# zjkang/Relation-DETR

Measured on AMD Instinct MI355X. Metric: images/sec @ 800×1333, 300 queries, R50 4-level; achieved HBM GB/s, higher is better.
Workload: dtype bf16; 1 GPU; relation_detr_resnet50_800_1333 transformer stack from feature pyramids: 6 encoder layers (MSDA self-attn, S=22323, 4 levels) + two-stage top-k + 6 decoder layers (relation-biased self-attn + MSDA cross-attn + box refinement) + top-300 detections; backbone/neck excluded; batch_per_gpu=4, global_batch=4, queries=900, levels=4, launch=hipGraph replay, streams=2, gemm_tuning=False, parallelism=image-parallel x1

## Files before the change

### relation_detr_amd/csrc/linear.hip

```cpp
#include <cstdlib>

#include "common.h"

namespace rdetr {

typedef __bf16 ln_bf16x8 __attribute__((ext_vector_type(8)));

constexpr int kLinK = 256;
constexpr int kLinThreads = 512;
constexpr int kLinRows = 32;

template <int NT, bool RELU>
__global__ __launch_bounds__(kLinThreads) void linear_k256_kernel(const uint16_t *__restrict__ x, long long ldx,
                                                                  const uint16_t *__restrict__ w, const uint16_t *__restrict__ bias,
                                                                  long long M, int N, uint16_t *__restrict__ out, long long ldo, int dbg,
                                                                  const unsigned char *__restrict__ row_mask, int hm_S)
{
    extern __shared__ __attribute__((aligned(16))) unsigned char lin_lds[];
    u32x4 *wl = reinterpret_cast<u32x4 *>(lin_lds);
    float *bl = reinterpret_cast<float *>(lin_lds + NT * 8 * 64 * 16);
    const int tid = threadIdx.x, lane = tid & 63, wave = tid >> 6;
    const int col = lane & 15, g = lane >> 4;
    const int n0 = blockIdx.y * (NT * 16);

    {
        constexpr int kPer = NT * 16 * 32 / kLinThreads;
        u32x4 piece[kPer];
#pragma unroll
        for (int i = 0; i < kPer; ++i) {
            const int idx = i * kLinThreads + tid, c = idx >> 5, p = idx & 31;
            piece[i] = n0 + c < N ? *reinterpret_cast<const u32x4 *>(w + (size_t)(n0 + c) * kLinK + 8 * p) : u32x4{0u, 0u, 0u, 0u};
        }
#pragma unroll
        for (int i = 0; i < kPer; ++i) {
            const int idx = i * kLinThreads + tid, c = idx >> 5, p = idx & 31;
            const int t = 2 * (c >> 5) + ((c >> 2) & 1), m = 4 * ((c >> 3) & 3) + (c & 3);
            wl[(t * 8 + (p >> 2)) * 64 + 16 * (p & 3) + m] = piece[i];
        }
    }
    for (int i = tid; i < NT * 16; i += kLinThreads) bl[i] = (bias && n0 + i < N) ? bf16_bits_to_f32(bias[n0 + i]) : 0.f;
    __syncthreads();

    const long long nsteps = (M + kLinRows - 1) / kLinRows;
    constexpr int kWaves = kLinThreads / 64;
    const long long stride = (long long)gridDim.x * kWaves;
    long long step = (long long)blockIdx.x * kWaves + wave;

    u32x4 xc[2][8], xn[2][8];
    auto load_rows = [&](long long st, u32x4 (&dst)[2][8]) {
#pragma unroll
        for (int cb = 0; cb < 2; ++cb) {
            const long long row = st * kLinRows + cb * 16 + col;
            const uint16_t *p = x + row * ldx + 8 * g;
#pragma unroll
            for (int s = 0; s < 8; ++s)
                dst[cb][s] = (st < nsteps && row < M) ? *reinterpret_cast<const u32x4 *>(p + 32 * s) : u32x4{0u, 0u, 0u, 0u};
        }
    };
    load_rows(step, xc);
    for (; step < nsteps; step += stride) {
        load_rows(step + stride, xn);
        const long long row_a = step * kLinRows + col, row_b = row_a + 16;
        uint16_t *oa = out + row_a * ldo + n0 + 8 * g, *ob = out + row_b * ldo + n0 + 8 * g;
        bool zero_a = false, zero_b = false;
        if (hm_S) {
            const unsigned ia = (unsigned)row_a / (unsigned)hm_S, ib = (unsigned)row_b / (unsigned)hm_S;
            oa = out + ((long long)ia * 8 * hm_S + (row_a - (long long)ia * hm_S)) * 32 + 8 * g;
            ob = out + ((long long)ib * 8 * hm_S + (row_b - (long long)ib * hm_S)) * 32 + 8 * g;
            if (row_mask) {
                zero_a = row_a < M && row_mask[row_a] != 0;
                zero_b = row_b < M && row_mask[row_b] != 0;
            }
        }
#pragma unroll
        for (int u = 0; u < NT / 2; ++u) {
            f32x4 acc[2][2];
#pragma unroll
            for (int e = 0; e < 2; ++e) {
                const f32x4 b4 = *reinterpret_cast<const f32x4 *>(bl + 32 * u + 8 * g + 4 * e);
                acc[e][0] = b4;
                acc[e][1] = b4;
            }
            if (!(dbg & 2))
#pragma unroll
            for (int s = 0; s < 8; ++s) {
#pragma unroll
                for (int e = 0; e < 2; ++e) {
                    const ln_bf16x8 a = __builtin_bit_cast(ln_bf16x8, wl[((2 * u + e) * 8 + s) * 64 + lane]);
                    acc[e][0] = __builtin_amdgcn_mfma_f32_16x16x32_bf16(a, __builtin_bit_cast(ln_bf16x8, xc[0][s]), acc[e][0], 0, 0, 0);
                    acc[e][1] = __builtin_amdgcn_mfma_f32_16x16x32_bf16(a, __builtin_bit_cast(ln_bf16x8, xc[1][s]), acc[e][1], 0, 0, 0);
                }
            }
            if (n0 + 32 * u + 8 * g < N) {
#pragma unroll
                for (int cb = 0; cb < 2; ++cb) {
                    f32x4 lo = acc[0][cb], hi = acc[1][cb];
                    if (RELU) {
                        lo.x = fmaxf(lo.x, 0.f); lo.y = fmaxf(lo.y, 0.f); lo.z = fmaxf(lo.z, 0.f); lo.w = fmaxf(lo.w, 0.f);
                        hi.x = fmaxf(hi.x, 0.f); hi.y = fmaxf(hi.y, 0.f); hi.z = fmaxf(hi.z, 0.f); hi.w = fmaxf(hi.w, 0.f);
                    }
                    u32x4 pk;
                    pk.x = f32_to_bf16_bits(lo.x) | (f32_to_bf16_bits(lo.y) << 16);
                    pk.y = f32_to_bf16_bits(lo.z) | (f32_to_bf16_bits(lo.w) << 16);
                    pk.z = f32_to_bf16_bits(hi.x) | (f32_to_bf16_bits(hi.y) << 16);
                    pk.w = f32_to_bf16_bits(hi.z) | (f32_to_bf16_bits(hi.w) << 16);
                    if ((cb ? zero_b : zero_a)) pk = u32x4{0u, 0u, 0u, 0u};
                    const long long col_off = hm_S ? (long long)u * hm_S * 32 : 32 * u;
                    if ((cb ? row_b : row_a) < M && !((dbg & 1) && pk.x != 0x12345u)) *reinterpret_cast<u32x4 *>((cb ? ob : oa) + col_off) = pk;
                }
            }
            __builtin_amdgcn_sched_barrier(0);
        }
#pragma unroll
        for (int cb = 0; cb < 2; ++cb)
#pragma unroll
            for (int s = 0; s < 8; ++s) xc[cb][s] = xn[cb][s];
    }
}

template <int NT, bool RELU>
static int linear_launch(const uint16_t *x, long long ldx, const uint16_t *w, const uint16_t *bias, long long M, int N,
                         uint16_t *out, long long ldo, int chunks, hipStream_t st, const unsigned char *row_mask = nullptr, int hm_S = 0)
{
    auto kern = linear_k256_kernel<NT, RELU>;
    constexpr int lds = NT * 8 * 64 * 16 + NT * 16 * 4;
    static const hipError_t attr = hipFuncSetAttribute(reinterpret_cast<const void *>(kern),
                                                       hipFuncAttributeMaxDynamicSharedMemorySize, lds);
    if (attr != hipSuccess) return RDETR_ERR_LAUNCH;
    const long long steps = (M + kLinRows - 1) / kLinRows;
    long long gx = (steps + kLinThreads / 64 - 1) / (kLinThreads / 64);
    const long long cap = 256 / chunks > 0 ? 256 / chunks : 1;
    if (gx > cap) gx = cap;
    hipLaunchKernelGGL(kern, dim3((unsigned)gx, (unsigned)chunks), dim3(kLinThreads), (size_t)lds, st, x, ldx, w, bias, M, N, out,
                       ldo, 0, row_mask, hm_S);
    return launch_status();
}


constexpr int kLnlThreads = 512;
constexpr int kLnlWaves = kLnlThreads / 64;

__global__ __launch_bounds__(256) void linear_pack_kernel(const uint16_t *__restrict__ w, u32x4 *__restrict__ packed)
{
    const int idx = blockIdx.x * 256 + threadIdx.x;
    if (idx >= 16 * 8 * 64) return;
    const int t = idx >> 9, s = (idx >> 6) & 7, l = idx & 63, m = l & 15, kb = l >> 4;
    const int n = 32 * (t >> 1) + 8 * (m >> 2) + 4 * (t & 1) + (m & 3);
    packed[idx] = *reinterpret_cast<const u32x4 *>(w + (size_t)n * kLinK + 32 * s + 8 * kb);
}

__global__ __launch_bounds__(kLnlThreads) void linear_ln_k256_kernel(const uint16_t *__restrict__ x, long long ldx,
                                                                     const uint16_t *__restrict__ packed,
                                                                     const uint16_t *__restrict__ bias,
                                                                     const uint16_t *__restrict__ res, long long ldr,
                                                                     const uint16_t *__restrict__ gamma,
                                                                     const uint16_t *__restrict__ beta, float eps, long long M,
                                                                     uint16_t *__restrict__ out, long long ldo)
{
    extern __shared__ __attribute__((aligned(16))) unsigned char lin_lds[];
    const u32x4 *wl = reinterpret_cast<const u32x4 *>(lin_lds);
    float *bl = reinterpret_cast<float *>(lin_lds + 16 * 8 * 64 * 16);
    const int tid = threadIdx.x, lane = tid & 63, wave = __builtin_amdgcn_readfirstlane(tid >> 6);
    const int col = lane & 15, g = lane >> 4;
    {
        const unsigned lane_off = (unsigned)lane * 16u;
#pragma unroll 1
        for (int i = 0; i < 128 / kLnlWaves; ++i) {
            const int f = wave * (128 / kLnlWaves) + i;
            const unsigned m0v = (unsigned)f * 1024u;
            const unsigned char *src = reinterpret_cast<const unsigned char *>(packed) + f * 1024;
            asm volatile("s_mov_b32 m0, %0\n\ts_nop 0\n\tglobal_load_lds_dwordx4 %1, %2" : : "s"(m0v), "v"(lane_off), "s"(src) : "memory", "m0");
        }
    }
    if (tid < 256) {
        bl[tid] = bias ? bf16_bits_to_f32(bias[tid]) : 0.f;
        bl[256 + tid] = bf16_bits_to_f32(gamma[tid]);
        bl[512 + tid] = bf16_bits_to_f32(beta[tid]);
    }
    const long long nsteps = (M + kLinRows - 1) / kLinRows;
    long long step = (long long)blockIdx.x * kLnlWaves + wave;
    const long long stride = (long long)gridDim.x * kLnlWaves;
    asm volatile("s_waitcnt vmcnt(0)" ::: "memory");
    __syncthreads();
    for (; step < nsteps; step += stride) {
        const long long row_a = step * kLinRows + col, row_b = row_a + 16;
        u32x4 xc[2][8];
#pragma unroll
        for (int s = 0; s < 8; ++s) {
            xc[0][s] = row_a < M ? *reinterpret_cast<const u32x4 *>(x + row_a * ldx + 32 * s + 8 * g) : u32x4{0u, 0u, 0u, 0u};
            xc[1][s] = row_b < M ? *reinterpret_cast<const u32x4 *>(x + row_b * ldx + 32 * s + 8 * g) : u32x4{0u, 0u, 0u, 0u};
        }
        f32x4 acc[16][2];
        {
            auto frag = [&](int i) -> u32x4 { return wl[((i & 15) * 8 + (i >> 4)) * 64 + lane]; };
            const f32x4 zero4 = {0.f, 0.f, 0.f, 0.f};
            u32x4 ring[3];
            ring[0] = frag(0);
            ring[1] = frag(1);
#pragma unroll
            for (int i = 0; i < 128; ++i) {
                if (i + 2 < 128) ring[(i + 2) % 3] = frag(i + 2);
                __builtin_amdgcn_sched_barrier(0);
                const int s = i >> 4, t = i & 15;
                const ln_bf16x8 a = __builtin_bit_cast(ln_bf16x8, ring[i % 3]);
                acc[t][0] = __builtin_amdgcn_mfma_f32_16x16x32_bf16(a, __builtin_bit_cast(ln_bf16x8, xc[0][s]), s ? acc[t][0] : zero4, 0, 0, 0);
                acc[t][1] = __builtin_amdgcn_mfma_f32_16x16x32_bf16(a, __builtin_bit_cast(ln_bf16x8, xc[1][s]), s ? acc[t][1] : zero4, 0, 0, 0);
                __builtin_amdgcn_sched_barrier(0);
            }
        }
#pragma unroll
        for (int cb = 0; cb < 2; ++cb) {
            const long long row = cb ? row_b : row_a;
            const bool ok = row < M;
            float sum = 0.f;
#pragma unroll
            for (int u = 0; u < 8; ++u) {
                const u32x4 r = ok ? *reinterpret_cast<const u32x4 *>(res + row * ldr + 32 * u + 8 * g) : u32x4{0u, 0u, 0u, 0u};
                f32x4 &lo = acc[2 * u][cb], &hi = acc[2 * u + 1][cb];
                lo += *reinterpret_cast<const f32x4 *>(bl + 32 * u + 8 * g);
                hi += *reinterpret_cast<const f32x4 *>(bl + 32 * u + 8 * g + 4);
                const unsigned p0 = pack_bf16x2(lo.x, lo.y), p1 = pack_bf16x2(lo.z, lo.w), p2 = pack_bf16x2(hi.x, hi.y), p3 = pack_bf16x2(hi.z, hi.w);
                lo.x = __builtin_bit_cast(float, p0 << 16) + __builtin_bit_cast(float, r.x << 16);
                lo.y = __builtin_bit_cast(float, p0 & 0xffff0000u) + __builtin_bit_cast(float, r.x & 0xffff0000u);
                lo.z = __builtin_bit_cast(float, p1 << 16) + __builtin_bit_cast(float, r.y << 16);
                lo.w = __builtin_bit_cast(float, p1 & 0xffff0000u) + __builtin_bit_cast(float, r.y & 0xffff0000u);
                hi.x = __builtin_bit_cast(float, p2 << 16) + __builtin_bit_cast(float, r.z << 16);
                hi.y = __builtin_bit_cast(float, p2 & 0xffff0000u) + __builtin_bit_cast(float, r.z & 0xffff0000u);
                hi.z = __builtin_bit_cast(float, p3 << 16) + __builtin_bit_cast(float, r.w << 16);
                hi.w = __builtin_bit_cast(float, p3 & 0xffff0000u) + __builtin_bit_cast(float, r.w & 0xffff0000u);
                sum += ((lo.x + lo.y) + (lo.z + lo.w)) + ((hi.x + hi.y) + (hi.z + hi.w));
            }
            sum += __shfl_xor(sum, 16, 64);
            sum += __shfl_xor(sum, 32, 64);
            const float mean = sum * (1.0f / 256.0f);
            float sq = 0.f;
#pragma unroll
            for (int u = 0; u < 8; ++u) {
                f32x4 &lo = acc[2 * u][cb], &hi = acc[2 * u + 1][cb];
                lo.x -= mean; lo.y -= mean; lo.z -= mean; lo.w -= mean;
                hi.x -= mean; hi.y -= mean; hi.z -= mean; hi.w -= mean;
                sq += ((lo.x * lo.x + lo.y * lo.y) + (lo.z * lo.z + lo.w * lo.w)) + ((hi.x * hi.x + hi.y * hi.y) + (hi.z * hi.z + hi.w * hi.w));
            }
            sq += __shfl_xor(sq, 16, 64);
            sq += __shfl_xor(sq, 32, 64);
            const float rstd = 1.0f / sqrtf(sq * (1.0f / 256.0f) + eps);
#pragma unroll
            for (int u = 0; u < 8; ++u) {
                const f32x4 lo = acc[2 * u][cb], hi = acc[2 * u + 1][cb];
                const float *gp = bl + 256 + 32 * u + 8 * g, *bp = bl + 512 + 32 * u + 8 * g;
                const f32x4 g0 = *reinterpret_cast<const f32x4 *>(gp), g1 = *reinterpret_cast<const f32x4 *>(gp + 4);
                const f32x4 c0 = *reinterpret_cast<const f32x4 *>(bp), c1 = *reinterpret_cast<const f32x4 *>(bp + 4);
                u32x4 pk;
                pk.x = pack_bf16x2(lo.x * rstd * g0.x + c0.x, lo.y * rstd * g0.y + c0.y);
                pk.y = pack_bf16x2(lo.z * rstd * g0.z + c0.z, lo.w * rstd * g0.w + c0.w);
                pk.z = pack_bf16x2(hi.x * rstd * g1.x + c1.x, hi.y * rstd * g1.y + c1.y);
                pk.w = pack_bf16x2(hi.z * rstd * g1.z + c1.z, hi.w * rstd * g1.w + c1.w);
                if (ok) *reinterpret_cast<u32x4 *>(out + row * ldo + 32 * u + 8 * g) = pk;
            }
        }
    }
}

}

using namespace rdetr;

extern "C" int rdetr_linear_k256_bf16(const uint16_t *x, long long ldx, const uint16_t *w, const uint16_t *bias, long long M,
                                      int N, int relu, uint16_t *out, long long ldo, void *stream)
{
    if (M < 0 || N <= 0 || ldx < kLinK || ldo < N) return RDETR_ERR_INVALID_ARG;
    if ((N & 31) || (ldx & 7) || (ldo & 7)) return RDETR_ERR_UNSUPPORTED;
    if (M == 0) return RDETR_OK;
    if (!x || !w || !out) return RDETR_ERR_INVALID_ARG;
    if ((reinterpret_cast<uintptr_t>(x) | reinterpret_cast<uintptr_t>(w) | reinterpret_cast<uintptr_t>(out)) & 15) return RDETR_ERR_UNSUPPORTED;
    hipStream_t st = static_cast<hipStream_t>(stream);
    if (N % 256 == 0 || N < 192 || (N % 192 != 0)) {
        const int chunks = (N + 255) / 256;
        return relu ? linear_launch<16, true>(x, ldx, w, bias, M, N, out, ldo, chunks, st)
                    : linear_launch<16, false>(x, ldx, w, bias, M, N, out, ldo, chunks, st);
    }
    const int chunks = N / 192;
    return relu ? linear_launch<12, true>(x, ldx, w, bias, M, N, out, ldo, chunks, st)
                : linear_launch<12, false>(x, ldx, w, bias, M, N, out, ldo, chunks, st);
}

extern "C" int rdetr_linear_k256_hm_bf16(const uint16_t *x, long long ldx, const uint16_t *w, const uint16_t *bias,
                                         const uint8_t *row_mask, int B, int S, uint16_t *out_hm, void *stream)
{
    if (B < 0 || S < 0 || ldx < kLinK) return RDETR_ERR_INVALID_ARG;
    if (ldx & 7) return RDETR_ERR_UNSUPPORTED;
    if (B == 0 || S == 0) return RDETR_OK;
    if ((long long)B * S >= (1ll << 31)) return RDETR_ERR_UNSUPPORTED;
    if (!x || !w || !out_hm) return RDETR_ERR_INVALID_ARG;
    if ((reinterpret_cast<uintptr_t>(x) | reinterpret_cast<uintptr_t>(w) | reinterpret_cast<uintptr_t>(out_hm)) & 15) return RDETR_ERR_UNSUPPORTED;
    return linear_launch<16, false>(x, ldx, w, bias, (long long)B * S, 256, out_hm, 256, 1, static_cast<hipStream_t>(stream), row_mask, S);
}

extern "C" int rdetr_linear_pack_k256_bf16(const uint16_t *w, uint16_t *packed, void *stream)
{
    if (!w || !packed) return RDETR_ERR_INVALID_ARG;
    if ((reinterpret_cast<uintptr_t>(w) | reinterpret_cast<uintptr_t>(packed)) & 15) return RDETR_ERR_UNSUPPORTED;
    hipLaunchKernelGGL(linear_pack_kernel, dim3(32), dim3(256), 0, static_cast<hipStream_t>(stream), w, reinterpret_cast<u32x4 *>(packed));
    return launch_status();
}

extern "C" int rdetr_linear_ln_k256_bf16(const uint16_t *x, long long ldx, const uint16_t *packed, const uint16_t *bias,
                                         const uint16_t *residual, long long ldr, const uint16_t *gamma, const uint16_t *beta,
                                         float eps, long long M, uint16_t *out, long long ldo, void *stream)
{
    if (M < 0 || ldx < kLinK || ldr < kLinK || ldo < kLinK) return RDETR_ERR_INVALID_ARG;
    if ((ldx & 7) || (ldr & 7) || (ldo & 7)) return RDETR_ERR_UNSUPPORTED;
    if (M == 0) return RDETR_OK;
    if (!x || !packed || !residual || !gamma || !beta || !out) return RDETR_ERR_INVALID_ARG;
    if ((reinterpret_cast<uintptr_t>(x) | reinterpret_cast<uintptr_t>(packed) | reinterpret_cast<uintptr_t>(residual) |
         reinterpret_cast<uintptr_t>(out)) & 15)
        return RDETR_ERR_UNSUPPORTED;
    constexpr int lds = 16 * 8 * 64 * 16 + 3 * 256 * 4;
    static const hipError_t attr = hipFuncSetAttribute(reinterpret_cast<const void *>(linear_ln_k256_kernel),
                                                       hipFuncAttributeMaxDynamicSharedMemorySize, lds);
    if (attr != hipSuccess) return RDETR_ERR_LAUNCH;
    const long long steps = (M + kLinRows - 1) / kLinRows;
    long long gx = (steps + kLnlWaves - 1) / kLnlWaves;
    if (gx > 256) gx = 256;
    hipLaunchKernelGGL(linear_ln_k256_kernel, dim3((unsigned)gx), dim3(kLnlThreads), (size_t)lds, static_cast<hipStream_t>(stream), x,
                       ldx, packed, bias, residual, ldr, gamma, beta, eps, M, out, ldo);
    return launch_status();
}
```

### relation_detr_amd/csrc/proj.hip

```cpp
#include <type_traits>

#include "common.h"

namespace rdetr {

namespace {

typedef __bf16 pj_bf16x8 __attribute__((ext_vector_type(8)));

constexpr int kPjHalf = 8 * 8 * 64 * 16;
constexpr int kPjLdsBias = kPjHalf;
constexpr int kPjLdsBytes = kPjLdsBias + (256 + 512) * 4;

template <int CB, int THREADS, int QCOLS>
__global__ __launch_bounds__(THREADS) void encoder_proj_k256_kernel(
    const uint16_t *__restrict__ x, long long ldx, const uint16_t *__restrict__ xq, long long ldq, const uint16_t *__restrict__ pwv,
    const uint16_t *__restrict__ bv, const uint16_t *__restrict__ pwq, const uint16_t *__restrict__ bq,
    const unsigned char *__restrict__ row_mask, int S, long long M, uint16_t *__restrict__ out_hm, uint16_t *__restrict__ out_q)
{
    constexpr int kMaxFrags = CB == 2 ? 8 : 8;
    extern __shared__ __attribute__((aligned(16))) unsigned char pj_lds[];
    const u32x4 *wl = reinterpret_cast<const u32x4 *>(pj_lds);
    float *bl = reinterpret_cast<float *>(pj_lds + kPjLdsBias);
    const int tid = threadIdx.x, lane = tid & 63, wave = __builtin_amdgcn_readfirstlane(tid >> 6);
    const int nwaves = (int)(blockDim.x >> 6);
    const int col = lane & 15, g = lane >> 4;

    u32x4 stg[kMaxFrags];
    auto fetch = [&](const uint16_t *packed, int h) {
#pragma unroll
        for (int i = 0; i < kMaxFrags; ++i) {
            const int f = wave + i * nwaves;
            if (f < 64) stg[i] = reinterpret_cast<const u32x4 *>(packed)[((size_t)h * kPjHalf + (size_t)f * 1024) / 16 + lane];
        }
        __builtin_amdgcn_sched_barrier(0);
    };
    auto commit = [&]() {
        __syncthreads();
        u32x4 *dst = reinterpret_cast<u32x4 *>(pj_lds);
#pragma unroll
        for (int i = 0; i < kMaxFrags; ++i) {
            const int f = wave + i * nwaves;
            if (f < 64) dst[f * 64 + lane] = stg[i];
        }
        __syncthreads();
    };

    fetch(pwv, 0);
    for (int i = tid; i < 256; i += (int)blockDim.x) bl[i] = bv ? bf16_bits_to_f32(bv[i]) : 0.f;
    for (int i = tid; i < 512; i += (int)blockDim.x) bl[256 + i] = (bq && i < QCOLS) ? bf16_bits_to_f32(bq[i]) : 0.f;

    const long long row0 = ((long long)blockIdx.x * nwaves + wave) * (16 * CB) + col;
    u32x4 xr[CB][8], qr[CB][8];
    bool rok[CB], zero[CB];
    uint16_t *ohm[CB], *oq[CB];
#pragma unroll
    for (int cb = 0; cb < CB; ++cb) {
        const long long row = row0 + 16 * cb;
        rok[cb] = row < M;
        const long long r = rok[cb] ? row : 0;
#pragma unroll
        for (int s = 0; s < 8; ++s) {
            xr[cb][s] = rok[cb] ? *reinterpret_cast<const u32x4 *>(x + r * ldx + 32 * s + 8 * g) : u32x4{0u, 0u, 0u, 0u};
            qr[cb][s] = rok[cb] ? *reinterpret_cast<const u32x4 *>(xq + r * ldq + 32 * s + 8 * g) : u32x4{0u, 0u, 0u, 0u};
        }
        zero[cb] = rok[cb] && row_mask && row_mask[r] != 0;
        const long long img = r / S, pos = r - img * S;
        ohm[cb] = out_hm + ((img * 8) * (long long)S + pos) * 32 + 8 * g;
        oq[cb] = out_q + r * QCOLS + 8 * g;
    }

    auto mm = [&](const u32x4 &a, const u32x4 &bq_, const f32x4 &c) {
        return __builtin_amdgcn_mfma_f32_16x16x32_bf16(__builtin_bit_cast(pj_bf16x8, a), __builtin_bit_cast(pj_bf16x8, bq_), c, 0, 0, 0);
    };
    auto block = [&](const u32x4 (&xin)[CB][8], f32x4 (&acc)[4][2][CB], auto nfrags) {
        constexpr int kFrags = decltype(nfrags)::value, kAhead = 3;
        u32x4 ring[4];
        auto frag = [&](int f) { return wl[(((2 * (f >> 4) + (f & 1)) * 8 + ((f >> 1) & 7)) * 64) + lane]; };
#pragma unroll
        for (int f = 0; f < kAhead; ++f) ring[f & 3] = frag(f);
        const f32x4 zero4 = {0.f, 0.f, 0.f, 0.f};
#pragma unroll
        for (int f = 0; f < kFrags; ++f) {
            if (f + kAhead < kFrags) ring[(f + kAhead) & 3] = frag(f + kAhead);
            __builtin_amdgcn_sched_barrier(0);
#pragma unroll
            for (int cb = 0; cb < CB; ++cb)
                acc[f >> 4][f & 1][cb] = mm(ring[f & 3], xin[cb][(f >> 1) & 7], ((f >> 1) & 7) ? acc[f >> 4][f & 1][cb] : zero4);
            __builtin_amdgcn_sched_barrier(0);
        }
    };
    auto packed_out = [&](const f32x4 (&acc)[4][2][CB], const float *bias, int uu, int cb) {
        const f32x4 lo = acc[uu][0][cb] + *reinterpret_cast<const f32x4 *>(bias + 32 * uu + 8 * g);
        const f32x4 hi = acc[uu][1][cb] + *reinterpret_cast<const f32x4 *>(bias + 32 * uu + 8 * g + 4);
        return u32x4{pack_bf16x2(lo.x, lo.y), pack_bf16x2(lo.z, lo.w), pack_bf16x2(hi.x, hi.y), pack_bf16x2(hi.z, hi.w)};
    };

    constexpr int kBlocks = 2 + (QCOLS + 127) / 128;
    constexpr int kLastUnits = (QCOLS - 128 * (kBlocks - 3)) / 32;
    f32x4 acc[4][2][CB];
    commit();
#pragma unroll
    for (int p = 0; p < kBlocks; ++p) {
        if (p == 0) fetch(pwv, 1);
        else if (p < kBlocks - 1) fetch(pwq, p - 1);
        if (p < 2) {
            block(xr, acc, std::integral_constant<int, 64>{});
#pragma unroll
            for (int cb = 0; cb < CB; ++cb)
                if (rok[cb]) {
#pragma unroll
                    for (int uu = 0; uu < 4; ++uu) {
                        const u32x4 v = zero[cb] ? u32x4{0u, 0u, 0u, 0u} : packed_out(acc, bl + 128 * p, uu, cb);
                        *reinterpret_cast<u32x4 *>(ohm[cb] + (long long)(4 * p + uu) * S * 32) = v;
                    }
                }
        } else {
            constexpr int kUnitsOf[2] = {4, kLastUnits};
            const int units = kUnitsOf[p == kBlocks - 1];
            if (p == kBlocks - 1) block(qr, acc, std::integral_constant<int, 16 * kLastUnits>{});
            else block(qr, acc, std::integral_constant<int, 64>{});
#pragma unroll
            for (int cb = 0; cb < CB; ++cb)
                if (rok[cb]) {
#pragma unroll
                    for (int uu = 0; uu < 4; ++uu)
                        if (uu < units)
                            *reinterpret_cast<u32x4 *>(oq[cb] + 128 * (p - 2) + 32 * uu) = packed_out(acc, bl + 256 + 128 * (p - 2), uu, cb);
                }
        }
        if (p < kBlocks - 1) commit();
    }
}

}

}

using namespace rdetr;

extern "C" int rdetr_encoder_proj_k256_bf16(const uint16_t *x, long long ldx, const uint16_t *xq, long long ldq, const uint16_t *pwv,
                                            const uint16_t *bv, const uint16_t *pwq, const uint16_t *bq, const uint8_t *row_mask, int B, int S,
                                            int q_cols, uint16_t *out_hm, uint16_t *out_q, void *stream)
{
    if (B < 0 || S < 0 || ldx < 256 || ldq < 256) return RDETR_ERR_INVALID_ARG;
    if (q_cols != 384 && q_cols != 480) return RDETR_ERR_UNSUPPORTED;
    if ((ldx & 7) || (ldq & 7)) return RDETR_ERR_UNSUPPORTED;
    if (B == 0 || S == 0) return RDETR_OK;
    if (!x || !xq || !pwv || !pwq || !out_hm || !out_q) return RDETR_ERR_INVALID_ARG;
    auto al = [](const void *p) { return reinterpret_cast<uintptr_t>(p) % 16 == 0; };
    if (!al(x) || !al(xq) || !al(pwv) || !al(pwq) || !al(out_hm) || !al(out_q)) return RDETR_ERR_UNSUPPORTED;
    const long long M = (long long)B * S;
    static const hipError_t attr = [] {
        hipError_t e = hipSuccess;
        const void *fns[4] = {reinterpret_cast<const void *>(encoder_proj_k256_kernel<2, 512, 384>),
                              reinterpret_cast<const void *>(encoder_proj_k256_kernel<1, 768, 384>),
                              reinterpret_cast<const void *>(encoder_proj_k256_kernel<2, 512, 480>),
                              reinterpret_cast<const void *>(encoder_proj_k256_kernel<1, 768, 480>)};
        for (const void *fn : fns) {
            const hipError_t r = hipFuncSetAttribute(fn, hipFuncAttributeMaxDynamicSharedMemorySize, kPjLdsBytes);
            if (r != hipSuccess) e = r;
        }
        return e;
    }();
    if (attr != hipSuccess) return RDETR_ERR_LAUNCH;
    const auto rounds = [&](long long rows) { return ((M + rows - 1) / rows + 255) / 256; };
    long long best = 4 * rounds(256);
    int thin = 0;
#ifndef RDETR_PROJ_THIN
#define RDETR_PROJ_THIN 1
#endif
    if (RDETR_PROJ_THIN)
        for (int w = 12; w >= 9; --w) {
            const long long cost = 3 * rounds(16 * w);
            if (cost < best || (cost == best && thin)) {
                best = cost;
                thin = w;
            }
        }
    const long long tile_rows = thin ? 16 * thin : 256;
    const long long ntiles = (M + tile_rows - 1) / tile_rows;
    if (ntiles > 0x7fffffffll) return RDETR_ERR_UNSUPPORTED;
    hipStream_t st = static_cast<hipStream_t>(stream);
    auto launch = [&](auto kernel, unsigned threads) {
        hipLaunchKernelGGL(kernel, dim3((unsigned)ntiles), dim3(threads), kPjLdsBytes, st, x, ldx, xq, ldq, pwv, bv, pwq, bq, row_mask, S, M,
                           out_hm, out_q);
    };
    if (q_cols == 384) {
        if (thin) launch(encoder_proj_k256_kernel<1, 768, 384>, 64u * (unsigned)thin);
        else launch(encoder_proj_k256_kernel<2, 512, 384>, 512u);
    } else {
        if (thin) launch(encoder_proj_k256_kernel<1, 768, 480>, 64u * (unsigned)thin);
        else launch(encoder_proj_k256_kernel<2, 512, 480>, 512u);
    }
    return launch_status();
}
```

Measured before the change: 1090 images/s.

## Add thin one-tile-per-wave linear+LayerNorm kernel and double-buffer encoder projection weights

```diff
diff --git a/relation_detr_amd/csrc/linear.hip b/relation_detr_amd/csrc/linear.hip
--- a/relation_detr_amd/csrc/linear.hip
+++ b/relation_detr_amd/csrc/linear.hip
@@ -1,6 +1,7 @@
 #include <cstdlib>
 
 #include "common.h"
+#include "row_tiles.h"
 
 namespace rdetr {
 
@@ -149,49 +150,123 @@
     packed[idx] = *reinterpret_cast<const u32x4 *>(w + (size_t)n * kLinK + 32 * s + 8 * kb);
 }
 
+#ifdef RDETR_DEV
+static int g_lnl_dbg = 0;
+#endif
+
+__device__ __forceinline__ void lnl_finish_block(f32x4 (&acc)[16], const u32x4 (&r)[8], const float *bl, int g, float eps, bool ok,
+                                                 uint16_t *orow, int dbg)
+{
+    if (dbg & 8) {
+#pragma unroll
+        for (int u = 0; u < 8; ++u) {
+            const f32x4 lo = acc[2 * u], hi = acc[2 * u + 1];
+            const u32x4 pk = {pack_bf16x2(lo.x, lo.y) ^ r[u].x, pack_bf16x2(lo.z, lo.w) ^ r[u].y, pack_bf16x2(hi.x, hi.y) ^ r[u].z,
+                              pack_bf16x2(hi.z, hi.w) ^ r[u].w};
+            if (ok && !((dbg & 16) && pk.x != 0x12345u)) *reinterpret_cast<u32x4 *>(orow + 32 * u) = pk;
+        }
+        return;
+    }
+    float sum = 0.f;
+#pragma unroll
+    for (int u = 0; u < 8; ++u) {
+        f32x4 &lo = acc[2 * u], &hi = acc[2 * u + 1];
+        lo += *reinterpret_cast<const f32x4 *>(bl + 32 * u + 8 * g);
+        hi += *reinterpret_cast<const f32x4 *>(bl + 32 * u + 8 * g + 4);
+        const unsigned p0 = pack_bf16x2(lo.x, lo.y), p1 = pack_bf16x2(lo.z, lo.w), p2 = pack_bf16x2(hi.x, hi.y), p3 = pack_bf16x2(hi.z, hi.w);
+        lo.x = __builtin_bit_cast(float, p0 << 16) + __builtin_bit_cast(float, r[u].x << 16);
+        lo.y = __builtin_bit_cast(float, p0 & 0xffff0000u) + __builtin_bit_cast(float, r[u].x & 0xffff0000u);
+        lo.z = __builtin_bit_cast(float, p1 << 16) + __builtin_bit_cast(float, r[u].y << 16);
+        lo.w = __builtin_bit_cast(float, p1 & 0xffff0000u) + __builtin_bit_cast(float, r[u].y & 0xffff0000u);
+        hi.x = __builtin_bit_cast(float, p2 << 16) + __builtin_bit_cast(float, r[u].z << 16);
+        hi.y = __builtin_bit_cast(float, p2 & 0xffff0000u) + __builtin_bit_cast(float, r[u].z & 0xffff0000u);
+        hi.z = __builtin_bit_cast(float, p3 << 16) + __builtin_bit_cast(float, r[u].w << 16);
+        hi.w = __builtin_bit_cast(float, p3 & 0xffff0000u) + __builtin_bit_cast(float, r[u].w & 0xffff0000u);
+        sum += ((lo.x + lo.y) + (lo.z + lo.w)) + ((hi.x + hi.y) + (hi.z + hi.w));
+    }
+    sum += __shfl_xor(sum, 16, 64);
+    sum += __shfl_xor(sum, 32, 64);
+    const float mean = sum * (1.0f / 256.0f);
+    float sq = 0.f;
+#pragma unroll
+    for (int u = 0; u < 8; ++u) {
+        f32x4 &lo = acc[2 * u], &hi = acc[2 * u + 1];
+        lo.x -= mean; lo.y -= mean; lo.z -= mean; lo.w -= mean;
+        hi.x -= mean; hi.y -= mean; hi.z -= mean; hi.w -= mean;
+        sq += ((lo.x * lo.x + lo.y * lo.y) + (lo.z * lo.z + lo.w * lo.w)) + ((hi.x * hi.x + hi.y * hi.y) + (hi.z * hi.z + hi.w * hi.w));
+    }
+    sq += __shfl_xor(sq, 16, 64);
+    sq += __shfl_xor(sq, 32, 64);
+    const float rstd = 1.0f / sqrtf(sq * (1.0f / 256.0f) + eps);
+#pragma unroll
+    for (int u = 0; u < 8; ++u) {
+        const f32x4 lo = acc[2 * u], hi = acc[2 * u + 1];
+        const float *gp = bl + 256 + 32 * u + 8 * g, *bp = bl + 512 + 32 * u + 8 * g;
+        const f32x4 g0 = *reinterpret_cast<const f32x4 *>(gp), g1 = *reinterpret_cast<const f32x4 *>(gp + 4);
+        const f32x4 c0 = *reinterpret_cast<const f32x4 *>(bp), c1 = *reinterpret_cast<const f32x4 *>(bp + 4);
+        u32x4 pk;
+        pk.x = pack_bf16x2(lo.x * rstd * g0.x + c0.x, lo.y * rstd * g0.y + c0.y);
+        pk.y = pack_bf16x2(lo.z * rstd * g0.z + c0.z, lo.w * rstd * g0.w + c0.w);
+        pk.z = pack_bf16x2(hi.x * rstd * g1.x + c1.x, hi.y * rstd * g1.y + c1.y);
+        pk.w = pack_bf16x2(hi.z * rstd * g1.z + c1.z, hi.w * rstd * g1.w + c1.w);
+        if (ok && !((dbg & 16) && pk.x != 0x12345u)) *reinterpret_cast<u32x4 *>(orow + 32 * u) = pk;
+    }
+}
+
+__device__ __forceinline__ void lnl_fill_weights(const uint16_t *packed, int first, int end, int step, int lane)
+{
+    const unsigned lane_off = (unsigned)lane * 16u;
+#pragma unroll 1
+    for (int f = first; f < end; f += step) {
+        const unsigned m0v = (unsigned)f * 1024u;
+        const unsigned char *src = reinterpret_cast<const unsigned char *>(packed) + f * 1024;
+        asm volatile("s_mov_b32 m0, %0\n\ts_nop 0\n\tglobal_load_lds_dwordx4 %1, %2" : : "s"(m0v), "v"(lane_off), "s"(src) : "memory", "m0");
+    }
+}
+
 __global__ __launch_bounds__(kLnlThreads) void linear_ln_k256_kernel(const uint16_t *__restrict__ x, long long ldx,
                                                                      const uint16_t *__restrict__ packed,
                                                                      const uint16_t *__restrict__ bias,
                                                                      const uint16_t *__restrict__ res, long long ldr,
                                                                      const uint16_t *__restrict__ gamma,
                                                                      const uint16_t *__restrict__ beta, float eps, long long M,
-                                                                     uint16_t *__restrict__ out, long long ldo)
-{
+                                                                     uint16_t *__restrict__ out, long long ldo, int dbg_arg)
+{
+#ifdef RDETR_DEV
+    const int dbg = dbg_arg;
+#else
+    constexpr int dbg = 0;
+#endif
     extern __shared__ __attribute__((aligned(16))) unsigned char lin_lds[];
     const u32x4 *wl = reinterpret_cast<const u32x4 *>(lin_lds);
     float *bl = reinterpret_cast<float *>(lin_lds + 16 * 8 * 64 * 16);
     const int tid = threadIdx.x, lane = tid & 63, wave = __builtin_amdgcn_readfirstlane(tid >> 6);
     const int col = lane & 15, g = lane >> 4;
-    {
-        const unsigned lane_off = (unsigned)lane * 16u;
-#pragma unroll 1
-        for (int i = 0; i < 128 / kLnlWaves; ++i) {
-            const int f = wave * (128 / kLnlWaves) + i;
-            const unsigned m0v = (unsigned)f * 1024u;
-            const unsigned char *src = reinterpret_cast<const unsigned char *>(packed) + f * 1024;
-            asm volatile("s_mov_b32 m0, %0\n\ts_nop 0\n\tglobal_load_lds_dwordx4 %1, %2" : : "s"(m0v), "v"(lane_off), "s"(src) : "memory", "m0");
-        }
-    }
+    const long long nsteps = (M + kLinRows - 1) / kLinRows;
+    long long step = (long long)blockIdx.x * kLnlWaves + wave;
+    const long long stride = (long long)gridDim.x * kLnlWaves;
+    u32x4 xc[2][8];
+    auto load_x = [&](long long st) {
+        const long long row_a = st * kLinRows + col, row_b = row_a + 16;
+#pragma unroll
+        for (int s = 0; s < 8; ++s) {
+            xc[0][s] = (row_a < M && !(dbg & 2)) ? *reinterpret_cast<const u32x4 *>(x + row_a * ldx + 32 * s + 8 * g) : u32x4{0u, 0u, 0u, 0u};
+            xc[1][s] = (row_b < M && !(dbg & 2)) ? *reinterpret_cast<const u32x4 *>(x + row_b * ldx + 32 * s + 8 * g) : u32x4{0u, 0u, 0u, 0u};
+        }
+    };
+    if (!(dbg & 1)) lnl_fill_weights(packed, wave * (128 / kLnlWaves), (wave + 1) * (128 / kLnlWaves), 1, lane);
     if (tid < 256) {
         bl[tid] = bias ? bf16_bits_to_f32(bias[tid]) : 0.f;
         bl[256 + tid] = bf16_bits_to_f32(gamma[tid]);
         bl[512 + tid] = bf16_bits_to_f32(beta[tid]);
     }
-    const long long nsteps = (M + kLinRows - 1) / kLinRows;
-    long long step = (long long)blockIdx.x * kLnlWaves + wave;
-    const long long stride = (long long)gridDim.x * kLnlWaves;
     asm volatile("s_waitcnt vmcnt(0)" ::: "memory");
-    __syncthreads();
+    if (!(dbg & 32)) __syncthreads();
     for (; step < nsteps; step += stride) {
         const long long row_a = step * kLinRows + col, row_b = row_a + 16;
-        u32x4 xc[2][8];
-#pragma unroll
-        for (int s = 0; s < 8; ++s) {
-            xc[0][s] = row_a < M ? *reinterpret_cast<const u32x4 *>(x + row_a * ldx + 32 * s + 8 * g) : u32x4{0u, 0u, 0u, 0u};
-            xc[1][s] = row_b < M ? *reinterpret_cast<const u32x4 *>(x + row_b * ldx + 32 * s + 8 * g) : u32x4{0u, 0u, 0u, 0u};
-        }
-        f32x4 acc[16][2];
-        {
+        load_x(step);
+        f32x4 acc[2][16];
+        if (!(dbg & 4)) {
             auto frag = [&](int i) -> u32x4 { return wl[((i & 15) * 8 + (i >> 4)) * 64 + lane]; };
             const f32x4 zero4 = {0.f, 0.f, 0.f, 0.f};
             u32x4 ring[3];
@@ -203,67 +278,100 @@
                 __builtin_amdgcn_sched_barrier(0);
                 const int s = i >> 4, t = i & 15;
                 const ln_bf16x8 a = __builtin_bit_cast(ln_bf16x8, ring[i % 3]);
-                acc[t][0] = __builtin_amdgcn_mfma_f32_16x16x32_bf16(a, __builtin_bit_cast(ln_bf16x8, xc[0][s]), s ? acc[t][0] : zero4, 0, 0, 0);
-                acc[t][1] = __builtin_amdgcn_mfma_f32_16x16x32_bf16(a, __builtin_bit_cast(ln_bf16x8, xc[1][s]), s ? acc[t][1] : zero4, 0, 0, 0);
+                acc[0][t] = __builtin_amdgcn_mfma_f32_16x16x32_bf16(a, __builtin_bit_cast(ln_bf16x8, xc[0][s]), s ? acc[0][t] : zero4, 0, 0, 0);
+                acc[1][t] = __builtin_amdgcn_mfma_f32_16x16x32_bf16(a, __builtin_bit_cast(ln_bf16x8, xc[1][s]), s ? acc[1][t] : zero4, 0, 0, 0);
                 __builtin_amdgcn_sched_barrier(0);
+            }
+        } else {
+#pragma unroll
+            for (int t = 0; t < 16; ++t) {
+                acc[0][t] = __builtin_bit_cast(f32x4, xc[0][t & 7]);
+                acc[1][t] = __builtin_bit_cast(f32x4, xc[1][t & 7]);
             }
         }
 #pragma unroll
         for (int cb = 0; cb < 2; ++cb) {
             const long long row = cb ? row_b : row_a;
             const bool ok = row < M;
-            float sum = 0.f;
-#pragma unroll
-            for (int u = 0; u < 8; ++u) {
-                const u32x4 r = ok ? *reinterpret_cast<const u32x4 *>(res + row * ldr + 32 * u + 8 * g) : u32x4{0u, 0u, 0u, 0u};
-                f32x4 &lo = acc[2 * u][cb], &hi = acc[2 * u + 1][cb];
-                lo += *reinterpret_cast<const f32x4 *>(bl + 32 * u + 8 * g);
-                hi += *reinterpret_cast<const f32x4 *>(bl + 32 * u + 8 * g + 4);
-                const unsigned p0 = pack_bf16x2(lo.x, lo.y), p1 = pack_bf16x2(lo.z, lo.w), p2 = pack_bf16x2(hi.x, hi.y), p3 = pack_bf16x2(hi.z, hi.w);
-                lo.x = __builtin_bit_cast(float, p0 << 16) + __builtin_bit_cast(float, r.x << 16);
-                lo.y = __builtin_bit_cast(float, p0 & 0xffff0000u) + __builtin_bit_cast(float, r.x & 0xffff0000u);
-                lo.z = __builtin_bit_cast(float, p1 << 16) + __builtin_bit_cast(float, r.y << 16);
-                lo.w = __builtin_bit_cast(float, p1 & 0xffff0000u) + __builtin_bit_cast(float, r.y & 0xffff0000u);
-                hi.x = __builtin_bit_cast(float, p2 << 16) + __builtin_bit_cast(float, r.z << 16);
-                hi.y = __builtin_bit_cast(float, p2 & 0xffff0000u) + __builtin_bit_cast(float, r.z & 0xffff0000u);
-                hi.z = __builtin_bit_cast(float, p3 << 16) + __builtin_bit_cast(float, r.w << 16);
-                hi.w = __builtin_bit_cast(float, p3 & 0xffff0000u) + __builtin_bit_cast(float, r.w & 0xffff0000u);
-                sum += ((lo.x + lo.y) + (lo.z + lo.w)) + ((hi.x + hi.y) + (hi.z + hi.w));
-            }
-            sum += __shfl_xor(sum, 16, 64);
-            sum += __shfl_xor(sum, 32, 64);
-            const float mean = sum * (1.0f / 256.0f);
-            float sq = 0.f;
-#pragma unroll
-            for (int u = 0; u < 8; ++u) {
-                f32x4 &lo = acc[2 * u][cb], &hi = acc[2 * u + 1][cb];
-                lo.x -= mean; lo.y -= mean; lo.z -= mean; lo.w -= mean;
-                hi.x -= mean; hi.y -= mean; hi.z -= mean; hi.w -= mean;
-                sq += ((lo.x * lo.x + lo.y * lo.y) + (lo.z * lo.z + lo.w * lo.w)) + ((hi.x * hi.x + hi.y * hi.y) + (hi.z * hi.z + hi.w * hi.w));
-            }
-            sq += __shfl_xor(sq, 16, 64);
-            sq += __shfl_xor(sq, 32, 64);
-            const float rstd = 1.0f / sqrtf(sq * (1.0f / 256.0f) + eps);
-#pragma unroll
-            for (int u = 0; u < 8; ++u) {
-                const f32x4 lo = acc[2 * u][cb], hi = acc[2 * u + 1][cb];
-                const float *gp = bl + 256 + 32 * u + 8 * g, *bp = bl + 512 + 32 * u + 8 * g;
-                const f32x4 g0 = *reinterpret_cast<const f32x4 *>(gp), g1 = *reinterpret_cast<const f32x4 *>(gp + 4);
-                const f32x4 c0 = *reinterpret_cast<const f32x4 *>(bp), c1 = *reinterpret_cast<const f32x4 *>(bp + 4);
-                u32x4 pk;
-                pk.x = pack_bf16x2(lo.x * rstd * g0.x + c0.x, lo.y * rstd * g0.y + c0.y);
-                pk.y = pack_bf16x2(lo.z * rstd * g0.z + c0.z, lo.w * rstd * g0.w + c0.w);
-                pk.z = pack_bf16x2(hi.x * rstd * g1.x + c1.x, hi.y * rstd * g1.y + c1.y);
-                pk.w = pack_bf16x2(hi.z * rstd * g1.z + c1.z, hi.w * rstd * g1.w + c1.w);
-                if (ok) *reinterpret_cast<u32x4 *>(out + row * ldo + 32 * u + 8 * g) = pk;
-            }
-        }
-    }
+            u32x4 r[8];
+#pragma unroll
+            for (int u = 0; u < 8; ++u)
+                r[u] = (ok && !(dbg & 2)) ? *reinterpret_cast<const u32x4 *>(res + row * ldr + 32 * u + 8 * g) : u32x4{0u, 0u, 0u, 0u};
+            lnl_finish_block(acc[cb], r, bl, g, eps, ok, out + row * ldo + 8 * g, dbg);
+        }
+    }
+}
+
+__global__ __launch_bounds__(768) void linear_ln_k256_thin_kernel(const uint16_t *__restrict__ x, long long ldx,
+                                                                  const uint16_t *__restrict__ packed,
+                                                                  const uint16_t *__restrict__ bias,
+                                                                  const uint16_t *__restrict__ res, long long ldr,
+                                                                  const uint16_t *__restrict__ gamma,
+                                                                  const uint16_t *__restrict__ beta, float eps, long long M,
+                                                                  uint16_t *__restrict__ out, long long ldo, int dbg_arg)
+{
+#ifdef RDETR_DEV
+    const int dbg = dbg_arg;
+#else
+    constexpr int dbg = 0;
+#endif
+    extern __shared__ __attribute__((aligned(16))) unsigned char lin_lds[];
+    const u32x4 *wl = reinterpret_cast<const u32x4 *>(lin_lds);
+    float *bl = reinterpret_cast<float *>(lin_lds + 16 * 8 * 64 * 16);
+    const int tid = threadIdx.x, lane = tid & 63, wave = __builtin_amdgcn_readfirstlane(tid >> 6);
+    const int nwaves = __builtin_amdgcn_readfirstlane((int)(blockDim.x >> 6));
+    const int col = lane & 15, g = lane >> 4;
+    const long long row = ((long long)blockIdx.x * nwaves + wave) * 16 + col;
+    const bool ok = row < M;
+    const long long rowc = ok ? row : M - 1;
+    u32x4 xc[8], r[8];
+#pragma unroll
+    for (int s = 0; s < 8; ++s) xc[s] = r[s] = u32x4{0u, 0u, 0u, 0u};
+    if (!(dbg & 2))
+#pragma unroll
+        for (int s = 0; s < 8; ++s) xc[s] = *reinterpret_cast<const u32x4 *>(x + rowc * ldx + 32 * s + 8 * g);
+    if (!(dbg & 1)) lnl_fill_weights(packed, wave, 128, nwaves, lane);
+    for (int i = tid; i < 256; i += (int)blockDim.x) {
+        bl[i] = bias ? bf16_bits_to_f32(bias[i]) : 0.f;
+        bl[256 + i] = bf16_bits_to_f32(gamma[i]);
+        bl[512 + i] = bf16_bits_to_f32(beta[i]);
+    }
+    asm volatile("s_waitcnt vmcnt(0)" ::: "memory");
+    if (!(dbg & 32)) __syncthreads();
+    if (!(dbg & 2))
+#pragma unroll
+        for (int u = 0; u < 8; ++u) r[u] = *reinterpret_cast<const u32x4 *>(res + rowc * ldr + 32 * u + 8 * g);
+    __builtin_amdgcn_sched_barrier(0);
+    f32x4 acc[16];
+    if (!(dbg & 4)) {
+        auto frag = [&](int i) -> u32x4 { return wl[((i & 15) * 8 + (i >> 4)) * 64 + lane]; };
+        const f32x4 zero4 = {0.f, 0.f, 0.f, 0.f};
+        u32x4 ring[4];
+#pragma unroll
+        for (int i = 0; i < 3; ++i) ring[i] = frag(i);
+#pragma unroll
+        for (int i = 0; i < 128; ++i) {
+            if (i + 3 < 128) ring[(i + 3) & 3] = frag(i + 3);
+            __builtin_amdgcn_sched_barrier(0);
+            const int s = i >> 4, t = i & 15;
+            acc[t] = __builtin_amdgcn_mfma_f32_16x16x32_bf16(__builtin_bit_cast(ln_bf16x8, ring[i & 3]), __builtin_bit_cast(ln_bf16x8, xc[s]),
+                                                             s ? acc[t] : zero4, 0, 0, 0);
+            __builtin_amdgcn_sched_barrier(0);
+        }
+    } else {
+#pragma unroll
+        for (int t = 0; t < 16; ++t) acc[t] = __builtin_bit_cast(f32x4, xc[t & 7]);
+    }
+    lnl_finish_block(acc, r, bl, g, eps, ok, out + row * ldo + 8 * g, dbg);
 }
 
 }
 
 using namespace rdetr;
+
+#ifdef RDETR_DEV
+extern "C" void rdetr_dev_set_linear_ln_dbg(int v) { rdetr::g_lnl_dbg = v; }
+#endif
 
 extern "C" int rdetr_linear_k256_bf16(const uint16_t *x, long long ldx, const uint16_t *w, const uint16_t *bias, long long M,
                                       int N, int relu, uint16_t *out, long long ldo, void *stream)
@@ -316,13 +424,30 @@
          reinterpret_cast<uintptr_t>(out)) & 15)
         return RDETR_ERR_UNSUPPORTED;
     constexpr int lds = 16 * 8 * 64 * 16 + 3 * 256 * 4;
-    static const hipError_t attr = hipFuncSetAttribute(reinterpret_cast<const void *>(linear_ln_k256_kernel),
-                                                       hipFuncAttributeMaxDynamicSharedMemorySize, lds);
+    static const hipError_t attr = [] {
+        const hipError_t a = hipFuncSetAttribute(reinterpret_cast<const void *>(linear_ln_k256_kernel), hipFuncAttributeMaxDynamicSharedMemorySize, lds);
+        const hipError_t b = hipFuncSetAttribute(reinterpret_cast<const void *>(linear_ln_k256_thin_kernel), hipFuncAttributeMaxDynamicSharedMemorySize, lds);
+        return a != hipSuccess ? a : b;
+    }();
     if (attr != hipSuccess) return RDETR_ERR_LAUNCH;
+#ifdef RDETR_DEV
+    const int dbg = g_lnl_dbg;
+#else
+    const int dbg = 0;
+#endif
+#ifndef RDETR_LNL_THIN
+#define RDETR_LNL_THIN 1
+#endif
+    const RowTiles tiles = choose_row_tiles(M, RDETR_LNL_THIN != 0);
+    if (RDETR_LNL_THIN == 2 ? tiles.thin_waves && tiles.rounds == 1 : RDETR_LNL_THIN && linear_ln_thin_pays(M)) {
+        hipLaunchKernelGGL(linear_ln_k256_thin_kernel, dim3((unsigned)tiles.ntiles), dim3(64u * (unsigned)tiles.thin_waves), (size_t)lds,
+                           static_cast<hipStream_t>(stream), x, ldx, packed, bias, residual, ldr, gamma, beta, eps, M, out, ldo, dbg);
+        return launch_status();
+    }
     const long long steps = (M + kLinRows - 1) / kLinRows;
     long long gx = (steps + kLnlWaves - 1) / kLnlWaves;
     if (gx > 256) gx = 256;
     hipLaunchKernelGGL(linear_ln_k256_kernel, dim3((unsigned)gx), dim3(kLnlThreads), (size_t)lds, static_cast<hipStream_t>(stream), x,
-                       ldx, packed, bias, residual, ldr, gamma, beta, eps, M, out, ldo);
+                       ldx, packed, bias, residual, ldr, gamma, beta, eps, M, out, ldo, dbg);
     return launch_status();
 }
diff --git a/relation_detr_amd/csrc/proj.hip b/relation_detr_amd/csrc/proj.hip
--- a/relation_detr_amd/csrc/proj.hip
+++ b/relation_detr_amd/csrc/proj.hip
@@ -1,6 +1,7 @@
 #include <type_traits>
 
 #include "common.h"
+#include "row_tiles.h"
 
 namespace rdetr {
 
@@ -9,72 +10,95 @@
 typedef __bf16 pj_bf16x8 __attribute__((ext_vector_type(8)));
 
 constexpr int kPjHalf = 8 * 8 * 64 * 16;
-constexpr int kPjLdsBias = kPjHalf;
+constexpr int kPjLdsBias = 2 * kPjHalf;
 constexpr int kPjLdsBytes = kPjLdsBias + (256 + 512) * 4;
+
+#ifdef RDETR_DEV
+int g_pj_dbg = 0;
+#endif
 
 template <int CB, int THREADS, int QCOLS>
 __global__ __launch_bounds__(THREADS) void encoder_proj_k256_kernel(
     const uint16_t *__restrict__ x, long long ldx, const uint16_t *__restrict__ xq, long long ldq, const uint16_t *__restrict__ pwv,
     const uint16_t *__restrict__ bv, const uint16_t *__restrict__ pwq, const uint16_t *__restrict__ bq,
-    const unsigned char *__restrict__ row_mask, int S, long long M, uint16_t *__restrict__ out_hm, uint16_t *__restrict__ out_q)
+    const unsigned char *__restrict__ row_mask, int S, long long M, uint16_t *__restrict__ out_hm, uint16_t *__restrict__ out_q, int dbg_arg)
 {
-    constexpr int kMaxFrags = CB == 2 ? 8 : 8;
+#ifdef RDETR_DEV
+    const int dbg = dbg_arg;
+#else
+    constexpr int dbg = 0;
+#endif
     extern __shared__ __attribute__((aligned(16))) unsigned char pj_lds[];
-    const u32x4 *wl = reinterpret_cast<const u32x4 *>(pj_lds);
     float *bl = reinterpret_cast<float *>(pj_lds + kPjLdsBias);
     const int tid = threadIdx.x, lane = tid & 63, wave = __builtin_amdgcn_readfirstlane(tid >> 6);
-    const int nwaves = (int)(blockDim.x >> 6);
+    const int nwaves = __builtin_amdgcn_readfirstlane((int)(blockDim.x >> 6));
     const int col = lane & 15, g = lane >> 4;
-
-    u32x4 stg[kMaxFrags];
-    auto fetch = [&](const uint16_t *packed, int h) {
-#pragma unroll
-        for (int i = 0; i < kMaxFrags; ++i) {
-            const int f = wave + i * nwaves;
-            if (f < 64) stg[i] = reinterpret_cast<const u32x4 *>(packed)[((size_t)h * kPjHalf + (size_t)f * 1024) / 16 + lane];
-        }
-        __builtin_amdgcn_sched_barrier(0);
-    };
-    auto commit = [&]() {
-        __syncthreads();
-        u32x4 *dst = reinterpret_cast<u32x4 *>(pj_lds);
-#pragma unroll
-        for (int i = 0; i < kMaxFrags; ++i) {
-            const int f = wave + i * nwaves;
-            if (f < 64) dst[f * 64 + lane] = stg[i];
-        }
-        __syncthreads();
-    };
-
-    fetch(pwv, 0);
-    for (int i = tid; i < 256; i += (int)blockDim.x) bl[i] = bv ? bf16_bits_to_f32(bv[i]) : 0.f;
-    for (int i = tid; i < 512; i += (int)blockDim.x) bl[256 + i] = (bq && i < QCOLS) ? bf16_bits_to_f32(bq[i]) : 0.f;
+    constexpr int kBlocks = 2 + (QCOLS + 127) / 128;
+    constexpr int kLastUnits = (QCOLS - 128 * (kBlocks - 3)) / 32;
+
+    auto fill = [&](int p) {
+        if (dbg & 1) return;
+        const unsigned char *slab = reinterpret_cast<const unsigned char *>(p < 2 ? pwv : pwq) + (size_t)(p < 2 ? p : p - 2) * kPjHalf;
+        const unsigned buf = (unsigned)(p & 1) * (unsigned)kPjHalf, lane_off = (unsigned)lane * 16u;
+#pragma unroll 1
+        for (int f = wave; f < 64; f += nwaves) {
+            const unsigned m0v = buf + (unsigned)f * 1024u;
+            const unsigned char *src = slab + f * 1024;
+            asm volatile("s_mov_b32 m0, %0\n\ts_nop 0\n\tglobal_load_lds_dwordx4 %1, %2" : : "s"(m0v), "v"(lane_off), "s"(src) : "memory", "m0");
+        }
+    };
+    fill(0);
+    fill(1);
 
     const long long row0 = ((long long)blockIdx.x * nwaves + wave) * (16 * CB) + col;
     u32x4 xr[CB][8], qr[CB][8];
     bool rok[CB], zero[CB];
+    long long rr[CB];
     uint16_t *ohm[CB], *oq[CB];
 #pragma unroll
     for (int cb = 0; cb < CB; ++cb) {
         const long long row = row0 + 16 * cb;
         rok[cb] = row < M;
-        const long long r = rok[cb] ? row : 0;
-#pragma unroll
-        for (int s = 0; s < 8; ++s) {
-            xr[cb][s] = rok[cb] ? *reinterpret_cast<const u32x4 *>(x + r * ldx + 32 * s + 8 * g) : u32x4{0u, 0u, 0u, 0u};
-            qr[cb][s] = rok[cb] ? *reinterpret_cast<const u32x4 *>(xq + r * ldq + 32 * s + 8 * g) : u32x4{0u, 0u, 0u, 0u};
-        }
+        rr[cb] = rok[cb] ? row : 0;
+#pragma unroll
+        for (int s = 0; s < 8; ++s) xr[cb][s] = qr[cb][s] = u32x4{0u, 0u, 0u, 0u};
+    }
+    if (!(dbg & 2))
+#pragma unroll
+        for (int cb = 0; cb < CB; ++cb)
+#pragma unroll
+            for (int s = 0; s < 8; ++s) xr[cb][s] = *reinterpret_cast<const u32x4 *>(x + rr[cb] * ldx + 32 * s + 8 * g);
+    for (int i = tid; i < 256; i += (int)blockDim.x) bl[i] = bv ? bf16_bits_to_f32(bv[i]) : 0.f;
+    for (int i = tid; i < 512; i += (int)blockDim.x) bl[256 + i] = (bq && i < QCOLS) ? bf16_bits_to_f32(bq[i]) : 0.f;
+#pragma unroll
+    for (int cb = 0; cb < CB; ++cb) {
+        const long long r = rr[cb];
         zero[cb] = rok[cb] && row_mask && row_mask[r] != 0;
         const long long img = r / S, pos = r - img * S;
         ohm[cb] = out_hm + ((img * 8) * (long long)S + pos) * 32 + 8 * g;
         oq[cb] = out_q + r * QCOLS + 8 * g;
     }
+    asm volatile("s_waitcnt vmcnt(0)" ::: "memory");
+    if (!(dbg & 32)) __syncthreads();
+    if (!(dbg & 2))
+#pragma unroll
+        for (int cb = 0; cb < CB; ++cb)
+#pragma unroll
+            for (int s = 0; s < 8; ++s) qr[cb][s] = *reinterpret_cast<const u32x4 *>(xq + rr[cb] * ldq + 32 * s + 8 * g);
+    __builtin_amdgcn_sched_barrier(0);
 
     auto mm = [&](const u32x4 &a, const u32x4 &bq_, const f32x4 &c) {
         return __builtin_amdgcn_mfma_f32_16x16x32_bf16(__builtin_bit_cast(pj_bf16x8, a), __builtin_bit_cast(pj_bf16x8, bq_), c, 0, 0, 0);
     };
-    auto block = [&](const u32x4 (&xin)[CB][8], f32x4 (&acc)[4][2][CB], auto nfrags) {
+    auto block = [&](const u32x4 *wl, const u32x4 (&xin)[CB][8], f32x4 (&acc)[4][2][CB], auto nfrags) {
         constexpr int kFrags = decltype(nfrags)::value, kAhead = 3;
+        if (dbg & 4) {
+#pragma unroll
+            for (int f = 0; f < 8; ++f)
+#pragma unroll
+                for (int cb = 0; cb < CB; ++cb) acc[f >> 1][f & 1][cb] = __builtin_bit_cast(f32x4, xin[cb][f]);
+            return;
+        }
         u32x4 ring[4];
         auto frag = [&](int f) { return wl[(((2 * (f >> 4) + (f & 1)) * 8 + ((f >> 1) & 7)) * 64) + lane]; };
 #pragma unroll
@@ -91,45 +115,50 @@
         }
     };
     auto packed_out = [&](const f32x4 (&acc)[4][2][CB], const float *bias, int uu, int cb) {
-        const f32x4 lo = acc[uu][0][cb] + *reinterpret_cast<const f32x4 *>(bias + 32 * uu + 8 * g);
-        const f32x4 hi = acc[uu][1][cb] + *reinterpret_cast<const f32x4 *>(bias + 32 * uu + 8 * g + 4);
+        f32x4 lo = acc[uu][0][cb], hi = acc[uu][1][cb];
+        if (!(dbg & 8)) {
+            lo += *reinterpret_cast<const f32x4 *>(bias + 32 * uu + 8 * g);
+            hi += *reinterpret_cast<const f32x4 *>(bias + 32 * uu + 8 * g + 4);
+        }
         return u32x4{pack_bf16x2(lo.x, lo.y), pack_bf16x2(lo.z, lo.w), pack_bf16x2(hi.x, hi.y), pack_bf16x2(hi.z, hi.w)};
     };
-
-    constexpr int kBlocks = 2 + (QCOLS + 127) / 128;
-    constexpr int kLastUnits = (QCOLS - 128 * (kBlocks - 3)) / 32;
+    auto store = [&](uint16_t *dst, const u32x4 &v) {
+        if (!((dbg & 16) && v.x != 0x12345u)) *reinterpret_cast<u32x4 *>(dst) = v;
+    };
+
     f32x4 acc[4][2][CB];
-    commit();
 #pragma unroll
     for (int p = 0; p < kBlocks; ++p) {
-        if (p == 0) fetch(pwv, 1);
-        else if (p < kBlocks - 1) fetch(pwq, p - 1);
+        const u32x4 *wl = reinterpret_cast<const u32x4 *>(pj_lds + (p & 1) * kPjHalf);
+        if (p < 2) block(wl, xr, acc, std::integral_constant<int, 64>{});
+        else if (p == kBlocks - 1) block(wl, qr, acc, std::integral_constant<int, 16 * kLastUnits>{});
+        else block(wl, qr, acc, std::integral_constant<int, 64>{});
+        if (p < kBlocks - 1) {
+            if (p >= 1) asm volatile("s_waitcnt vmcnt(0)" ::: "memory");
+            if (!(dbg & 32)) __syncthreads();
+            if (p + 2 < kBlocks) fill(p + 2);
+        }
         if (p < 2) {
-            block(xr, acc, std::integral_constant<int, 64>{});
 #pragma unroll
             for (int cb = 0; cb < CB; ++cb)
                 if (rok[cb]) {
 #pragma unroll
                     for (int uu = 0; uu < 4; ++uu) {
                         const u32x4 v = zero[cb] ? u32x4{0u, 0u, 0u, 0u} : packed_out(acc, bl + 128 * p, uu, cb);
-                        *reinterpret_cast<u32x4 *>(ohm[cb] + (long long)(4 * p + uu) * S * 32) = v;
+                        store(ohm[cb] + (long long)(4 * p + uu) * S * 32, v);
                     }
                 }
         } else {
             constexpr int kUnitsOf[2] = {4, kLastUnits};
             const int units = kUnitsOf[p == kBlocks - 1];
-            if (p == kBlocks - 1) block(qr, acc, std::integral_constant<int, 16 * kLastUnits>{});
-            else block(qr, acc, std::integral_constant<int, 64>{});
 #pragma unroll
             for (int cb = 0; cb < CB; ++cb)
                 if (rok[cb]) {
 #pragma unroll
                     for (int uu = 0; uu < 4; ++uu)
-                        if (uu < units)
-                            *reinterpret_cast<u32x4 *>(oq[cb] + 128 * (p - 2) + 32 * uu) = packed_out(acc, bl + 256 + 128 * (p - 2), uu, cb);
+                        if (uu < units) store(oq[cb] + 128 * (p - 2) + 32 * uu, packed_out(acc, bl + 256 + 128 * (p - 2), uu, cb));
                 }
         }
-        if (p < kBlocks - 1) commit();
     }
 }
 
@@ -138,6 +167,10 @@
 }
 
 using namespace rdetr;
+
+#ifdef RDETR_DEV
+extern "C" void rdetr_dev_set_proj_dbg(int v) { g_pj_dbg = v; }
+#endif
 
 extern "C" int rdetr_encoder_proj_k256_bf16(const uint16_t *x, long long ldx, const uint16_t *xq, long long ldq, const uint16_t *pwv,
                                             const uint16_t *bv, const uint16_t *pwq, const uint16_t *bq, const uint8_t *row_mask, int B, int S,
@@ -164,27 +197,22 @@
         return e;
     }();
     if (attr != hipSuccess) return RDETR_ERR_LAUNCH;
-    const auto rounds = [&](long long rows) { return ((M + rows - 1) / rows + 255) / 256; };
-    long long best = 4 * rounds(256);
-    int thin = 0;
 #ifndef RDETR_PROJ_THIN
 #define RDETR_PROJ_THIN 1
 #endif
-    if (RDETR_PROJ_THIN)
-        for (int w = 12; w >= 9; --w) {
-            const long long cost = 3 * rounds(16 * w);
-            if (cost < best || (cost == best && thin)) {
-                best = cost;
-                thin = w;
-            }
-        }
-    const long long tile_rows = thin ? 16 * thin : 256;
-    const long long ntiles = (M + tile_rows - 1) / tile_rows;
+    const RowTiles tiles = choose_row_tiles(M, RDETR_PROJ_THIN != 0);
+    const int thin = tiles.thin_waves;
+    const long long ntiles = tiles.ntiles;
     if (ntiles > 0x7fffffffll) return RDETR_ERR_UNSUPPORTED;
+#ifdef RDETR_DEV
+    const int dbg = g_pj_dbg;
+#else
+    const int dbg = 0;
+#endif
     hipStream_t st = static_cast<hipStream_t>(stream);
     auto launch = [&](auto kernel, unsigned threads) {
         hipLaunchKernelGGL(kernel, dim3((unsigned)ntiles), dim3(threads), kPjLdsBytes, st, x, ldx, xq, ldq, pwv, bv, pwq, bq, row_mask, S, M,
-                           out_hm, out_q);
+                           out_hm, out_q, dbg);
     };
     if (q_cols == 384) {
         if (thin) launch(encoder_proj_k256_kernel<1, 768, 384>, 64u * (unsigned)thin);
diff --git a/relation_detr_amd/csrc/row_tiles.h b/relation_detr_amd/csrc/row_tiles.h
--- /dev/null
+++ b/relation_detr_amd/csrc/row_tiles.h
@@ -0,0 +1,45 @@
+#pragma once
+
+namespace rdetr {
+
+struct RowTiles {
+    int thin_waves;
+    long long tile_rows, ntiles, rounds;
+};
+
+constexpr long long row_tile_rounds(long long M, long long rows) { return ((M + rows - 1) / rows + 255) / 256; }
+
+constexpr RowTiles choose_row_tiles(long long M, bool allow_thin = true)
+{
+    long long best = 4 * row_tile_rounds(M, 256);
+    int thin = 0;
+    if (allow_thin)
+        for (int w = 12; w >= 9; --w) {
+            const long long cost = 3 * row_tile_rounds(M, 16 * w);
+            if (cost < best || (cost == best && thin)) {
+                best = cost;
+                thin = w;
+            }
+        }
+    const long long rows = thin ? 16 * thin : 256;
+    return RowTiles{thin, rows, (M + rows - 1) / rows, row_tile_rounds(M, rows)};
+}
+
+constexpr bool linear_ln_thin_pays(long long M)
+{
+    const RowTiles t = choose_row_tiles(M);
+    return t.thin_waves != 0 && t.rounds == 1 && (M + 255) / 256 <= 128;
+}
+
+static_assert(choose_row_tiles(22323).thin_waves == 9 && choose_row_tiles(22323).ntiles == 156 && choose_row_tiles(22323).rounds == 1, "");
+static_assert(choose_row_tiles(44646).thin_waves == 11 && choose_row_tiles(44646).ntiles == 254 && choose_row_tiles(44646).rounds == 1, "");
+static_assert(choose_row_tiles(89292).thin_waves == 11 && choose_row_tiles(89292).ntiles == 508 && choose_row_tiles(89292).rounds == 2, "");
+static_assert(choose_row_tiles(408196).thin_waves == 12 && choose_row_tiles(408196).ntiles == 2127 && choose_row_tiles(408196).rounds == 9, "");
+static_assert(choose_row_tiles(1).thin_waves == 9 && choose_row_tiles(1).ntiles == 1 && choose_row_tiles(1).rounds == 1, "");
+static_assert(choose_row_tiles(44646, false).thin_waves == 0 && choose_row_tiles(44646, false).ntiles == 175, "");
+static_assert(choose_row_tiles(256 * 192 + 5).thin_waves == 0 && choose_row_tiles(256 * 192 + 5).ntiles == 193, "");
+static_assert(choose_row_tiles(256 * 256 + 5).thin_waves == 9 && choose_row_tiles(256 * 256 + 5).rounds == 2, "");
+static_assert(linear_ln_thin_pays(1) && linear_ln_thin_pays(3600) && linear_ln_thin_pays(22323) && linear_ln_thin_pays(128 * 256), "");
+static_assert(!linear_ln_thin_pays(128 * 256 + 1) && !linear_ln_thin_pays(44646) && !linear_ln_thin_pays(89292) && !linear_ln_thin_pays(408196), "");
+
+}
```

New measurement: 1071 images/s. 1.7% lower.
